# EasyVision-Ton/VMG

Hardware: AMD Instinct MI355X
Metric: LR-frames/s (train: forward+loss+backward+AdamW), VMG-REDS-few_levels 4x SR (higher is better)
Workload: dtype bf16; 1 GPU; VMG-REDS-few_levels train step, per-GPU batch 4x7x3x64x64 -> 4x SR (BASELINE configs[1]); global_batch=4, frames_per_clip=7, parallelism=dp1, launch=eager, recompute_chains=False, fp8_chains=False

## Files before the change

include/vmg_hip.h:

```cpp
#ifndef VMG_HIP_H
#define VMG_HIP_H

#include <stdint.h>

#ifdef __cplusplus
extern "C" {
#endif

#define VMG_F32 0
#define VMG_BF16 1

#define VMG_ACT_NONE 0
#define VMG_ACT_RELU 1
#define VMG_ACT_LRELU 2
#define VMG_ACT_GELU 3

#define VMG_CONV_GENERAL 0
#define VMG_CONV_KSPLIT 2
#define VMG_CONV_WS 3
#define VMG_CONV_LINEAR_WRES 4
#define VMG_CONV_WSTAT 6

const char* vmg_last_error(void);
int vmg_version(void);
// ... 131 lines not shown
int vmg_layernorm_bwd(int dtype, int ndy, const void* const* dy, const void* x, const float* mean, const float* rstd, const float* w,
                      const void* add, void* dx, float* dw, float* db, int64_t M, int C, void* ws, void* stream);

int vmg_space_depth_ln_fwd(int dtype, int mode, const void* x, const float* w, const float* b, void* y, float* mean, float* rstd, int N, int H,
                           int W, int cseg, float eps, void* stream);
int vmg_space_depth_ln_bwd(int dtype, int mode, const void* dy, const void* x, const float* mean, const float* rstd, const float* w, void* dx,
                           float* dw, float* db, int N, int H, int W, int cseg, void* ws, void* stream);

int64_t vmg_group_reduce_ws_bytes(void);
int vmg_group_reduce(int dtype, const void* a, const void* b, const void* c3, float* out, int G, int64_t R, int C, int mode, float scale,
                     float* ws, int64_t ws_bytes, void* stream);
int vmg_group_reduce3(int dtype, const void* a, const void* b0, const void* b1, const void* b2, float* out, int G, int64_t R, int C, float scale,
                      float* ws, int64_t ws_bytes, void* stream);
int vmg_tab_elementwise(int dtype, int op, const void* p0, const void* p1, const void* p2, const float* coef, const float* add, float s,
                        void* o0, void* o1, void* o2, int64_t rows, int64_t R, int C, void* stream);

#define VMG_GATE_TANH 0
#define VMG_GATE_SIGMOID_SYMM 1
#define VMG_GATE_RELU 2
#define VMG_GATE_GELU 3
#define VMG_GATE_SILU 4
int vmg_gate_fwd(int dtype, int form, int act, const void* a, const void* y, void* out, int64_t rows, int C, void* stream);
int vmg_gate_bwd(int dtype, int form, int act, const void* dout, const void* a, const void* y, void* da, void* dy, int64_t rows, int C, void* stream);
int vmg_gate_res_fwd(int dtype, int form, int act, const void* a, const void* y, const void* res, const float* coef, void* out, int64_t rows, int G,
                     int C, void* stream);
int vmg_gate_res_bwd(int dtype, int form, int act, const void* dout, const void* a, const void* y, const float* coef, void* da, void* dy,
                     int64_t rows, int G, int C, void* stream);

#define VMG_SHIFT_VECTOR 1
#define VMG_SHIFT_ELEMENT 2
int vmg_patch_shift_plan(int dtype, int Cs, int aligned16);
int vmg_patch_shift_fwd(int dtype, int sign, int act, const void* x, void* y, int N, int H, int W, int Cs, void* stream);
int vmg_patch_shift_bwd(int dtype, int sign, int act, const void* dy, const void* x, void* dx, int N, int H, int W, int Cs, void* stream);
int vmg_se_mlp2_fwd(const float* m, const float* w1, const float* b1, const float* w2, const float* b2, float* pre, float* out, int G, int C, int Hd,
                    void* stream);
int vmg_se_mlp2_bwd(const float* dout, const float* out, const float* m, const float* pre, const float* w1, const float* w2, float* dm, float* dw1,
                    float* db1, float* dw2, float* db2, float* ws, int G, int C, int Hd, float dm_scale, int accumulate, void* stream);
int vmg_group_reduce2(int dtype, const void* a, const void* b0, const void* b1, float* out, int G, int64_t R, int C, float scale, float* ws,
                      int64_t ws_bytes, void* stream);
int vmg_mix2_fwd(int dtype, const void* h, const void* w, const float* coef, void* y, int64_t rows, int64_t R, int C, void* stream);
int vmg_mix2_bwd(int dtype, const void* dy, const float* coef, const float* add, void* dh, void* dw, int64_t rows, int64_t R, int C, void* stream);

#define VMG_DWCONV_VECTOR 1
#define VMG_DWCONV_ELEMENT 2
#define VMG_DWCONV_PLAN_INTS 8
int vmg_dwconv3_plan(int dtype, int N, int H, int W, int C, int aligned16, int* plan);
int vmg_dwconv3_fwd(int dtype, int src_act, int out_act, const void* e, const float* w, const float* b, void* a, int N, int H, int W, int C, void* stream);
int vmg_dwconv3_bwd_data(int dtype, int src_act, int out_act, const void* da, const void* a, const void* e, const float* w, void* de, int N, int H, int W,
                         int C, void* stream);
int64_t vmg_dwconv3_wgrad_ws_bytes(int dtype, int N, int H, int W, int C);
int vmg_dwconv3_bwd_weight(int dtype, int src_act, int out_act, const void* da, const void* a, const void* e, float* dW, float* db, int N, int H, int W,
                           int C, int accumulate, void* ws, int64_t ws_bytes, void* stream);

int vmg_warp_bilinear_fwd(int dtype, const void* x, const float* flow, void* out, int N, int H, int W, int C, void* stream);
int vmg_warp_bilinear_bwd(int dtype, const void* x, const float* flow, const void* dy, void* dx_acc, float* dflow, int N, int H,
                          int W, int C, void* stream);
int vmg_warp_nearest_planes(const float* loc, const float* flow, float* out, int N, int K2, int H, int W, void* stream);
int vmg_flow_smooth(const float* in, float* out, int64_t planes, int H, int W, int r, int backward, void* stream);

int vmg_ltam_fwd(int dtype, const void* q, const void* const* keys, const void* const* vals, const float* loc, const float* rpe,
                 const float* decay, void* out, float* lse, int n, int h, int w, int c, int heads, int wh, int ww, int t, float scale,
                 void* stream);
int vmg_ltam_bwd(int dtype, const void* q, const void* const* keys, const void* const* vals, const float* loc, const float* rpe,
                 const float* decay, const void* out, const float* lse, const void* dout, void* dq, void* const* dk_acc,
                 void* const* dv_acc, float* drpe, int n, int h, int w, int c, int heads, int wh, int ww, int t, float scale,
                 void* stream);
int64_t vmg_ltam_tab_bytes(int t);
int vmg_ltam_fwd_tab(int dtype, const void* q, const void* const* keys, const void* const* vals, const float* loc, const float* rpe,
                     const float* decay, void* out, float* lse, int n, int h, int w, int c, int heads, int wh, int ww, int t, float scale,
                     void* ws, int64_t ws_bytes, void* stream);
int vmg_ltam_bwd_tab(int dtype, const void* q, const void* const* keys, const void* const* vals, const float* loc, const float* rpe,
                     const float* decay, const void* out, const float* lse, const void* dout, void* dq, void* const* dk_acc,
                     void* const* dv_acc, float* drpe, int n, int h, int w, int c, int heads, int wh, int ww, int t, float scale,
                     void* ws, int64_t ws_bytes, void* stream);

int vmg_ltam_max_fwd(int dtype, const void* q, const void* const* keys, const void* const* vals, const float* loc, void* out, int* idx,
                     float* score, int n, int h, int w, int c, int heads, int t, void* stream);
int vmg_ltam_max_bwd(int dtype, const void* q, const void* const* keys, const void* const* vals, const float* loc, const int* idx,
                     const void* dout, void* dq, void* const* dk_acc, void* const* dv_acc, int n, int h, int w, int c, int heads, int t,
                     void* stream);
int vmg_ltam_max_fwd_tab(int dtype, const void* q, const void* const* keys, const void* const* vals, const float* loc, void* out, int* idx,
                         float* score, int n, int h, int w, int c, int heads, int t, void* ws, int64_t ws_bytes, void* stream);
int vmg_ltam_max_bwd_tab(int dtype, const void* q, const void* const* keys, const void* const* vals, const float* loc, const int* idx,
                         const void* dout, void* dq, void* const* dk_acc, void* const* dv_acc, int n, int h, int w, int c, int heads, int t,
                         void* ws, int64_t ws_bytes, void* stream);

int vmg_prof_begin(vmg_ctx* ctx, int klass, int stride, int max_samples);
int vmg_prof_end(vmg_ctx* ctx, int64_t* launches_seen, int* samples, double* total_ms);
int vmg_prof_select_pixels(vmg_ctx* ctx, int64_t pixels);
double vmg_prof_null_interval_us(int reps, void* stream);

int vmg_morphfc_fwd(int axis, int chunk, const void* x, const void* relu_mask, const void* packed, const float* bias, void* out, void* tok_out,
                    int BT, int H, int W, int C, int Cp, int cout_tiles, int relu, float in_scale, float out_scale, void* stream);
int64_t vmg_morphfc_token_rows(int axis, int chunk, int BT, int H, int W);
enum { VMG_MORPHFC_PLAN_INTS = 8 };
int vmg_morphfc_plan(int axis, int chunk, int BT, int H, int W, int C, int Cp, int has_mask, int ncu, int* plan);
int64_t vmg_morph_token_rows(int axis, int chunk, int BT, int H, int W);
int vmg_morph_tokens_gather(int dtype, int axis, int chunk, const void* x, void* tok, int BT, int H, int W, int C, int Cp, int ld, void* stream);
int vmg_morph_tokens_scatter(int dtype, int axis, int chunk, const void* tok, void* out, int BT, int H, int W, int C, int Cp, int ld, void* stream);
int vmg_morph_tokens_route(int dtype, int chunk, int C, int ld, int aligned);

int vmg_win3d_attn_fwd(int dtype, const void* q, const void* kv, const float* bq, const float* bkv, const float* table, void* out, float* lse,
                       int B, int D, int H, int W, int C, int heads, int wt, int sd, int sh, int sw, void* stream);
int64_t vmg_win3d_attn_bwd_ws_bytes(int B, int D, int H, int W, int heads, int wt);
int vmg_win3d_attn_bwd(int dtype, const void* q, const void* kv, const float* bq, const float* bkv, const float* table, const void* out,
                       const float* lse, const void* d_out, void* dq, void* dkv, float* dtable, float* dbq, float* dbkv, void* ws, int B, int D, int H, int W,
// ... 122 lines not shown
```

vmg_amd/csrc/warp.hip:

```cpp
#include "common.h"

namespace {

__device__ __forceinline__ float unnorm_coord(float pix, float flow, int size) {
  const float g = __fadd_rn(pix, flow);
  const float denom = (float)(size - 1 > 1 ? size - 1 : 1);
  const float gn = __fsub_rn(__fdiv_rn(__fmul_rn(2.0f, g), denom), 1.0f);
  return __fmul_rn(__fdiv_rn(__fadd_rn(gn, 1.0f), 2.0f), (float)(size - 1));
}

__device__ __forceinline__ float clip_border(float v, int size, float* grad_mult) {
  const float hi = (float)(size - 1);
  if (v <= 0.f) { if (grad_mult) *grad_mult = 0.f; return 0.f; }
  if (v >= hi) { if (grad_mult) *grad_mult = 0.f; return hi; }
  if (grad_mult) *grad_mult = 1.f;
  return v;
}

template <typename T>
struct V16 {
  static constexpr int N = 16 / sizeof(T);
  T v[N];
};

// ... 58 lines not shown
    const float x1f = x0f + 1.f, y1f = y0f + 1.f;
    const float tx = ix - x0f, ty = iy - y0f;
    const float wnw = (x1f - ix) * (y1f - iy), wne = (ix - x0f) * (y1f - iy), wsw = (x1f - ix) * (iy - y0f), wse = (ix - x0f) * (iy - y0f);
    const bool vnw = y0 >= 0 && y0 < H && x0 >= 0 && x0 < W, vne = y0 >= 0 && y0 < H && x1 >= 0 && x1 < W;
    const bool vsw = y1 >= 0 && y1 < H && x0 >= 0 && x0 < W, vse = y1 >= 0 && y1 < H && x1 >= 0 && x1 < W;
    const long long ib = n * H * W * C;
    const long long onw = ib + ((long long)y0 * W + x0) * C, one = ib + ((long long)y0 * W + x1) * C;
    const long long osw = ib + ((long long)y1 * W + x0) * C, ose = ib + ((long long)y1 * W + x1) * C;
    float gix = 0.f, giy = 0.f;
    if constexpr (sizeof(T) == 2) {
      for (int cb = 0; cb < C; cb += 128) {
        const int cp = cb + 2 * lane;
        const bool in = cp < C;
        const long long own = pix * C;
        const int cl = in ? cp : 0;
        const wp_bf16x2 gp = *reinterpret_cast<const wp_bf16x2*>(dy + own + cl);
        const wp_bf16x2 xnw = *reinterpret_cast<const wp_bf16x2*>(x + (vnw ? onw : own) + cl), xne = *reinterpret_cast<const wp_bf16x2*>(x + (vne ? one : own) + cl);
        const wp_bf16x2 xsw = *reinterpret_cast<const wp_bf16x2*>(x + (vsw ? osw : own) + cl), xse = *reinterpret_cast<const wp_bf16x2*>(x + (vse ? ose : own) + cl);
        const float g0 = in ? (float)gp[0] : 0.f, g1 = in ? (float)gp[1] : 0.f;
        const int sl = lane >> 1;
        const float a0 = __shfl(g0, sl, 64), a1 = __shfl(g1, sl, 64), b0 = __shfl(g0, 32 + sl, 64), b1 = __shfl(g1, 32 + sl, 64);
        const float glo = (lane & 1) ? a1 : a0, ghi = (lane & 1) ? b1 : b0;
        const int clo = cb + lane, chi = cb + 64 + lane;
        auto corner = [&](long long o, float wgt, float sx, float sy, wp_bf16x2 xp) __attribute__((always_inline)) {
          if (clo < C) atomicAdd(dx_acc + o + clo, glo * wgt);
          if (chi < C) atomicAdd(dx_acc + o + chi, ghi * wgt);
          const float xv = (float)xp[0] * g0 + (float)xp[1] * g1;
          gix += xv * sx;
          giy += xv * sy;
        };
        if (vnw) corner(onw, wnw, -(1.f - ty), -(1.f - tx), xnw);
        if (vne) corner(one, wne, (1.f - ty), -tx, xne);
        if (vsw) corner(osw, wsw, -ty, (1.f - tx), xsw);
        if (vse) corner(ose, wse, ty, tx, xse);
      }
    } else {
      for (int c = lane; c < C; c += 64) {
        const float g = to_f32(dy[pix * C + c]);
        if (vnw) { atomicAdd(dx_acc + onw + c, g * wnw); const float xv = to_f32(x[onw + c]) * g; gix -= xv * (1.f - ty); giy -= xv * (1.f - tx); }
        if (vne) { atomicAdd(dx_acc + one + c, g * wne); const float xv = to_f32(x[one + c]) * g; gix += xv * (1.f - ty); giy -= xv * tx; }
        if (vsw) { atomicAdd(dx_acc + osw + c, g * wsw); const float xv = to_f32(x[osw + c]) * g; gix -= xv * ty; giy += xv * (1.f - tx); }
        if (vse) { atomicAdd(dx_acc + ose + c, g * wse); const float xv = to_f32(x[ose + c]) * g; gix += xv * ty; giy += xv * tx; }
      }
    }
    gix = wave_sum(gix);
    giy = wave_sum(giy);
    if (lane == 0) {
      dflow[pix * 2] = gix * gmx;
      dflow[pix * 2 + 1] = giy * gmy;
    }
  }
}

__global__ __launch_bounds__(256) void warp_nearest_planes_kernel(const float* __restrict__ loc, const float* __restrict__ flow,
                                                                  float* __restrict__ out, int N, int K2, int H, int W) {
  const long long total = (long long)N * H * W;
  for (long long pix = blockIdx.x * 256LL + threadIdx.x; pix < total; pix += (long long)gridDim.x * 256) {
    const int px = (int)(pix % W);
    const int py = (int)((pix / W) % H);
    const long long n = pix / ((long long)W * H);
    const float ix = clip_border(unnorm_coord((float)px, flow[pix * 2], W), W, nullptr);
    const float iy = clip_border(unnorm_coord((float)py, flow[pix * 2 + 1], H), H, nullptr);
    const int xn = (int)nearbyintf(ix), yn = (int)nearbyintf(iy);
    const bool ok = xn >= 0 && xn < W && yn >= 0 && yn < H;
    for (int k = 0; k < K2; ++k) {
      const long long plane = (n * K2 + k) * H * W;
      out[plane + (long long)py * W + px] = ok ? loc[plane + (long long)yn * W + xn] : 0.f;
    }
  }
}

int grid_for(long long total) {
  long long b = (total + 255) / 256;
  return (int)(b > 8192 ? 8192 : (b < 1 ? 1 : b));
}

__device__ __forceinline__ int fs_reflect(int p, int n) { return p < n ? p : 2 * (n - 1) - p; }

__global__ void flow_smooth_fwd_kernel(const float* __restrict__ in, float* __restrict__ out, long long planes, int H, int W, int r) {
  const long long total = planes * H * W;
  const float inv = 1.0f / (float)(r * r);
  for (long long i = blockIdx.x * (long long)blockDim.x + threadIdx.x; i < total; i += (long long)gridDim.x * blockDim.x) {
    const int x = (int)(i % W), y = (int)((i / W) % H);
    const float* pl = in + (i / ((long long)W * H)) * H * W;
    const int y0 = (y / r) * r, x0 = (x / r) * r;
    float s = 0.f;
    for (int dy = 0; dy < r; ++dy) {
      const float* row = pl + (long long)fs_reflect(y0 + dy, H) * W;
      for (int dx = 0; dx < r; ++dx) s += row[fs_reflect(x0 + dx, W)];
    }
    out[i] = s * inv;
  }
}

__global__ void flow_smooth_bwd_kernel(const float* __restrict__ dout, float* __restrict__ din, long long planes, int H, int W, int r) {
  const long long total = planes * H * W;
  const int hf = (H + r - 1) / r * r, wf = (W + r - 1) / r * r;
  const float inv = 1.0f / (float)(r * r);
  for (long long i = blockIdx.x * (long long)blockDim.x + threadIdx.x; i < total; i += (long long)gridDim.x * blockDim.x) {
    const int x = (int)(i % W), y = (int)((i / W) % H);
    const float* pl = dout + (i / ((long long)W * H)) * H * W;
    int py[2] = {y, 2 * (H - 1) - y}, px[2] = {x, 2 * (W - 1) - x};
    const int ny = (py[1] >= H && py[1] < hf) ? 2 : 1, nx = (px[1] >= W && px[1] < wf) ? 2 : 1;
    float acc = 0.f;
    for (int a = 0; a < ny; ++a) {
      const int y0 = (py[a] / r) * r;
      for (int b = 0; b < nx; ++b) {
        const int x0 = (px[b] / r) * r;
        float g = 0.f;
        for (int dy = 0; dy < r && y0 + dy < H; ++dy)
          for (int dx = 0; dx < r && x0 + dx < W; ++dx) g += pl[(long long)(y0 + dy) * W + x0 + dx];
        acc += g;
      }
    }
    din[i] = acc * inv;
  }
}

}

extern "C" int vmg_warp_bilinear_fwd(int dtype, const void* x, const float* flow, void* out, int N, int H, int W, int C, void* stream) {
  VMG_CHECK(dtype == VMG_F32 || dtype == VMG_BF16, "warp_fwd: bad dtype");
  VMG_CHECK(x && flow && out && N > 0 && H > 0 && W > 0 && C > 0, "warp_fwd: bad arguments");
  const int vn = dtype == VMG_BF16 ? 8 : 4;
  VMG_CHECK(C % vn == 0, "warp_fwd: C must be a multiple of %d", vn);
  VMG_CHECK(((uintptr_t)x | (uintptr_t)out) % 16 == 0, "warp_fwd: pointers must be 16-byte aligned");
  const long long total = (long long)N * H * W * (C / vn);
  hipStream_t st = (hipStream_t)stream;
  if (dtype == VMG_BF16) hipLaunchKernelGGL(warp_bilinear_fwd_kernel<bf16>, dim3(grid_for(total)), dim3(256), 0, st, (const bf16*)x, flow, (bf16*)out, N, H, W, C);
  else hipLaunchKernelGGL(warp_bilinear_fwd_kernel<float>, dim3(grid_for(total)), dim3(256), 0, st, (const float*)x, flow, (float*)out, N, H, W, C);
  VMG_LAUNCH_CHECK();
  return 0;
}

extern "C" int vmg_warp_bilinear_bwd(int dtype, const void* x, const float* flow, const void* dy, void* dx_acc, float* dflow, int N,
                                     int H, int W, int C, void* stream) {
  VMG_CHECK(dtype == VMG_F32 || dtype == VMG_BF16, "warp_bwd: bad dtype");
  VMG_CHECK(x && flow && dy && dx_acc && dflow && N > 0 && H > 0 && W > 0 && C > 0, "warp_bwd: bad arguments");
  const int vn = dtype == VMG_BF16 ? 8 : 4;
  VMG_CHECK(C % vn == 0, "warp_bwd: C must be a multiple of %d", vn);
  VMG_CHECK(((uintptr_t)x | (uintptr_t)dy | (uintptr_t)dx_acc) % 16 == 0, "warp_bwd: pointers must be 16-byte aligned");
  const long long total = (long long)N * H * W * 64;
  hipStream_t st = (hipStream_t)stream;
  if (dtype == VMG_BF16) {
    hipLaunchKernelGGL(warp_bilinear_bwd_kernel<bf16>, dim3(grid_for(total)), dim3(256), 0, st, (const bf16*)x, flow, (const bf16*)dy, (float*)dx_acc, dflow, N, H, W, C);
  } else {
    hipLaunchKernelGGL(warp_bilinear_bwd_kernel<float>, dim3(grid_for(total)), dim3(256), 0, st, (const float*)x, flow, (const float*)dy, (float*)dx_acc, dflow, N, H, W, C);
  }
  VMG_LAUNCH_CHECK();
  return 0;
}

extern "C" int vmg_warp_nearest_planes(const float* loc, const float* flow, float* out, int N, int K2, int H, int W, void* stream) {
  VMG_CHECK(loc && flow && out && N > 0 && K2 > 0 && H > 0 && W > 0, "warp_nearest: bad arguments");
  hipLaunchKernelGGL(warp_nearest_planes_kernel, dim3(grid_for((long long)N * H * W)), dim3(256), 0, (hipStream_t)stream, loc, flow, out, N, K2, H, W);
  VMG_LAUNCH_CHECK();
  return 0;
}

extern "C" int vmg_flow_smooth(const float* in, float* out, int64_t planes, int H, int W, int r, int backward, void* stream) {
  VMG_CHECK(in && out && planes > 0 && H > 0 && W > 0 && r >= 1, "flow_smooth: bad arguments");
  const int hf = (H + r - 1) / r * r, wf = (W + r - 1) / r * r;
  VMG_CHECK(hf - H < H && wf - W < W, "flow_smooth: the reflected padding must be smaller than the plane (as F.pad(mode='reflect') demands)");
  const long long total = planes * H * W;
  if (backward) hipLaunchKernelGGL(flow_smooth_bwd_kernel, dim3(grid_for(total)), dim3(256), 0, (hipStream_t)stream, in, out, (long long)planes, H, W, r);
  else hipLaunchKernelGGL(flow_smooth_fwd_kernel, dim3(grid_for(total)), dim3(256), 0, (hipStream_t)stream, in, out, (long long)planes, H, W, r);
  VMG_LAUNCH_CHECK();
  return 0;
}
```

vmg_amd/hip.py:

```python
from __future__ import annotations

import ctypes
import os
from ctypes import POINTER, c_char_p, c_float, c_int, c_int64, c_void_p

import torch

HERE = os.path.dirname(os.path.abspath(__file__))
LIB_PATH = os.environ.get("VMG_HIP_LIB") or os.path.join(HERE, "libvmg_hip.so")

F32, BF16 = 0, 1
ACT_NONE, ACT_RELU, ACT_LRELU, ACT_GELU = 0, 1, 2, 3
GATE_ACTS = {"tanh": 0, "sigmoid": 1, "relu": 2, "gelu": 3, "swish": 4}
SHIFT_VECTOR, SHIFT_ELEMENT = 1, 2
DWCONV_VECTOR, DWCONV_ELEMENT, DWCONV_PLAN_INTS = 1, 2, 8
CONV_GENERAL, CONV_KSPLIT, CONV_WS, CONV_LINEAR_WRES, CONV_WSTAT = 0, 2, 3, 4, 6
CONV_FAM_IGEMM, CONV_FAM_KSPLIT, CONV_FAM_WS, CONV_FAM_LINEAR_WRES, CONV_FAM_WSTAT = 1, 2, 3, 4, 5
CONV_PLAN_INTS = 11
MORPHFC_PLAN_INTS = 8
MORPH_ROUTE_ELEMENT, MORPH_ROUTE_LDS = 0, 1
WGRAD_V1, WGRAD_3, WGRAD_3B, WGRAD_L2, WGRAD_7 = 1, 2, 3, 4, 5


def wgrad_kernel_id(kind: int, a: int = 0, b: int = 0, c: int = 0) -> int:
    return kind << 24 | a << 16 | b << 8 | c


class HipError(RuntimeError):
    pass


class ConvDesc(ctypes.Structure):
    _fields_ = [
        ("dtype", c_int), ("ks", c_int), ("cout_tiles", c_int),
        ("N", c_int), ("H", c_int), ("W", c_int), ("Cout", c_int),
        ("nsrc", c_int),
        ("src", c_void_p * 4), ("src_ps", c_int64 * 4), ("src_ch", c_int * 4),
        ("packed", c_void_p), ("bias", c_void_p),
        ("out", c_void_p), ("out_ps", c_int64), ("out_pre", c_void_p),
        ("res", c_void_p), ("res_ps", c_int64),
        ("aux", c_void_p), ("aux_ps", c_int64),
        ("act", c_int), ("slope", c_float), ("alpha", c_float),
        ("actgrad", c_int), ("pixel_shuffle", c_int), ("mt", c_int), ("deep", c_int),
    ]


class ChainDesc(ctypes.Structure):
    _fields_ = [
        ("dtype", c_int), ("N", c_int), ("H", c_int), ("W", c_int), ("C", c_int), ("nblk", c_int), ("nsrc", c_int),
        ("src", c_void_p * 4), ("src_ps", c_int64 * 4), ("src_ch", c_int * 4),
        ("packed0", c_void_p), ("bias0", c_void_p), ("slope0", c_float), ("cout_tiles0", c_int), ("deep0", c_int),
        ("packed1", POINTER(c_void_p)), ("bias1", POINTER(c_void_p)), ("packed2", POINTER(c_void_p)), ("bias2", POINTER(c_void_p)),
        ("r_scaling", c_float), ("cout_tiles", c_int), ("deep", c_int),
        ("y", POINTER(c_void_p)), ("t", POINTER(c_void_p)), ("g_y", POINTER(c_void_p)), ("g_t", POINTER(c_void_p)),
    ]


class SpyModuleDesc(ctypes.Structure):
    _fields_ = [
        ("N", c_int), ("H", c_int), ("W", c_int),
        ("x", c_void_p), ("packed", c_void_p * 5), ("bias", c_void_p * 5), ("y", c_void_p * 4), ("out", c_void_p), ("dpre", c_void_p * 4),
    ]


class ConvQ8Desc(ctypes.Structure):
    _fields_ = [
        ("N", c_int), ("H", c_int), ("W", c_int), ("Cin", c_int), ("Cout", c_int),
        ("src", c_void_p), ("packed", c_void_p), ("bias", c_void_p),
        ("out", c_void_p), ("out_ps", c_int64), ("outq", c_void_p),
        ("res", c_void_p), ("res_ps", c_int64),
        ("act", c_int), ("slope", c_float), ("alpha", c_float),
    ]

# ... 35 lines not shown
                                  c_void_p, c_void_p]),
    "vmg_morphfc_fwd": (c_int, [c_int, c_int, c_void_p, c_void_p, c_void_p, c_void_p, c_void_p, c_void_p, c_int, c_int, c_int, c_int, c_int, c_int, c_int, c_float, c_float,
                                c_void_p]),
    "vmg_morphfc_token_rows": (c_int64, [c_int, c_int, c_int, c_int, c_int]),
    "vmg_morphfc_plan": (c_int, [c_int, c_int, c_int, c_int, c_int, c_int, c_int, c_int, c_int, POINTER(c_int)]),
    "vmg_morph_tokens_route": (c_int, [c_int, c_int, c_int, c_int, c_int]),
    "vmg_morph_token_rows": (c_int64, [c_int, c_int, c_int, c_int, c_int]),
    "vmg_morph_tokens_gather": (c_int, [c_int, c_int, c_int, c_void_p, c_void_p, c_int, c_int, c_int, c_int, c_int, c_int, c_void_p]),
    "vmg_morph_tokens_scatter": (c_int, [c_int, c_int, c_int, c_void_p, c_void_p, c_int, c_int, c_int, c_int, c_int, c_int, c_void_p]),
    "vmg_win3d_attn_fwd": (c_int, [c_int, c_void_p, c_void_p, c_void_p, c_void_p, c_void_p, c_void_p, c_void_p, c_int, c_int, c_int, c_int, c_int, c_int, c_int,
                                   c_int, c_int, c_int, c_void_p]),
    "vmg_win3d_attn_bwd": (c_int, [c_int, c_void_p, c_void_p, c_void_p, c_void_p, c_void_p, c_void_p, c_void_p, c_void_p, c_void_p, c_void_p, c_void_p, c_void_p,
                                   c_void_p, c_void_p, c_int, c_int, c_int, c_int, c_int, c_int, c_int, c_int, c_int, c_int, c_void_p]),
    "vmg_win3d_attn_bwd_ws_bytes": (c_int64, [c_int, c_int, c_int, c_int, c_int, c_int]),
    "vmg_conv_wgrad3_multi": (c_int, [c_int, c_int, c_void_p, c_void_p, c_int, c_int, c_int, c_int64, c_int, c_int64, c_int, c_void_p, c_int, c_int, c_int,
                                      c_void_p, c_void_p, c_void_p, c_int64, c_void_p]),
    "vmg_conv_wgrad3_variant": (c_int, [c_int]),
    "vmg_conv_wgrad_last_kernel": (c_int, []),
    "vmg_conv_wgrad_plan": (c_int, [c_int, c_int, c_int, c_int, c_int, c_int, c_int, c_int, c_int64, c_int, c_int64, c_int, c_int, c_int, c_int, c_int, c_int64,
                                    POINTER(c_int)]),
    "vmg_win3d_variant": (c_int, [c_int]),
    "vmg_linear_wgrad2_multi": (c_int, [c_int, c_int, c_void_p, c_void_p, c_int64, c_int64, c_int, c_int64, c_int, c_void_p, c_int, c_int, c_int,
                                        c_void_p, c_void_p, c_void_p, c_int64, c_void_p]),
    "vmg_replay_build": (c_void_p, [c_void_p, c_void_p, c_void_p]),
    "vmg_replay_kernel_info": (c_int, [c_void_p, c_int, c_void_p, c_void_p, c_void_p, c_void_p]),
    "vmg_replay_run": (c_int, [c_void_p, c_int, c_int, c_void_p]),
    "vmg_replay_destroy": (None, [c_void_p]),
    "vmg_pack_entry_bytes": (c_int, []),
    "vmg_pack_entry": (c_int, [c_void_p, c_int, c_int, c_void_p, c_int, c_int, c_int, c_int, c_int, c_int, c_void_p, c_void_p, c_int, c_int, c_void_p,
                               c_int]),
    "vmg_pack_run": (c_int, [c_void_p, c_int, c_int, c_void_p]),
    "vmg_group_reduce3": (c_int, [c_int, c_void_p, c_void_p, c_void_p, c_void_p, c_void_p, c_int, c_int64, c_int, ctypes.c_float, c_void_p, c_int64, c_void_p]),
    "vmg_group_reduce_ws_bytes": (c_int64, []),
    "vmg_se_mlp_fwd": (c_int, [c_void_p] * 7 + [c_int] * 6 + [c_void_p]),
    "vmg_se_mlp_bwd": (c_int, [c_void_p] * 12 + [c_int] * 6 + [ctypes.c_float, c_int, c_void_p]),
    "vmg_maxpool_fwd": (c_int, [c_int, c_void_p, c_void_p, c_void_p, c_int, c_int, c_int, c_int, c_int, c_void_p]),
    "vmg_maxpool_bwd": (c_int, [c_int, c_void_p, c_void_p, c_void_p, c_int, c_int, c_int, c_int, c_int, c_void_p]),
    "vmg_avgpool2_nhwc": (c_int, [c_int, c_void_p, c_void_p, c_int, c_int, c_int, c_int, c_void_p]),
    "vmg_upsample2x_ac_fwd": (c_int, [c_void_p, c_void_p, c_int, c_int, c_int, c_int, c_float, c_void_p]),
    "vmg_upsample2x_ac_bwd": (c_int, [c_void_p, c_void_p, c_int, c_int, c_int, c_int, c_float, c_void_p]),
    "vmg_spy_operand_fwd": (c_int, [c_int, c_void_p, c_void_p, c_void_p, c_void_p, c_int64, c_void_p]),
    "vmg_spy_operand_bwd": (c_int, [c_int, c_void_p, c_void_p, c_void_p, c_int64, c_void_p]),
    "vmg_spy_flow_add": (c_int, [c_int, c_void_p, c_void_p, c_void_p, c_int64, c_void_p]),
    "vmg_spy_prep": (c_int, [c_int, c_void_p, c_void_p, c_void_p, c_void_p, c_int64, c_int, c_int, c_void_p]),
    "vmg_spy_module_fwd": (c_int, [POINTER(SpyModuleDesc), c_void_p]),
    "vmg_spy_module_bwd": (c_int, [POINTER(SpyModuleDesc), c_void_p]),
    "vmg_space_depth_ln_fwd": (c_int, [c_int, c_int, c_void_p, c_void_p, c_void_p, c_void_p, c_void_p, c_void_p, c_int, c_int, c_int, c_int, c_float, c_void_p]),
    "vmg_space_depth_ln_bwd": (c_int, [c_int, c_int, c_void_p, c_void_p, c_void_p, c_void_p, c_void_p, c_void_p, c_void_p, c_void_p, c_int, c_int, c_int, c_int,
                                       c_void_p, c_void_p]),
    "vmg_conv_wgrad_batched": (c_int, [c_int, c_int, c_int, POINTER(c_void_p), POINTER(c_void_p), c_int, c_int, c_int, c_int64, c_int,
                                       c_int64, c_int, c_void_p, c_int, c_int, c_int, c_void_p, c_float, c_void_p]),
    "vmg_warp_bilinear_fwd": (c_int, [c_int, c_void_p, c_void_p, c_void_p, c_int, c_int, c_int, c_int, c_void_p]),
    "vmg_warp_bilinear_bwd": (c_int, [c_int, c_void_p, c_void_p, c_void_p, c_void_p, c_void_p, c_int, c_int, c_int, c_int, c_void_p]),
    "vmg_warp_nearest_planes": (c_int, [c_void_p, c_void_p, c_void_p, c_int, c_int, c_int, c_int, c_void_p]),
    "vmg_flow_smooth": (c_int, [c_void_p, c_void_p, c_int64, c_int, c_int, c_int, c_int, c_void_p]),
    "vmg_ltam_fwd": (c_int, [c_int, c_void_p, POINTER(c_void_p), POINTER(c_void_p), c_void_p, c_void_p, c_void_p, c_void_p, c_void_p,
                             c_int, c_int, c_int, c_int, c_int, c_int, c_int, c_int, c_float, c_void_p]),
    "vmg_ltam_bwd": (c_int, [c_int, c_void_p, POINTER(c_void_p), POINTER(c_void_p), c_void_p, c_void_p, c_void_p, c_void_p, c_void_p,
                             c_void_p, c_void_p, POINTER(c_void_p), POINTER(c_void_p), c_void_p, c_int, c_int, c_int, c_int, c_int,
                             c_int, c_int, c_int, c_float, c_void_p]),
    "vmg_ltam_tab_bytes": (c_int64, [c_int]),
    "vmg_ltam_fwd_tab": (c_int, [c_int, c_void_p, POINTER(c_void_p), POINTER(c_void_p), c_void_p, c_void_p, c_void_p, c_void_p, c_void_p,
                                 c_int, c_int, c_int, c_int, c_int, c_int, c_int, c_int, c_float, c_void_p, c_int64, c_void_p]),
    "vmg_ltam_bwd_tab": (c_int, [c_int, c_void_p, POINTER(c_void_p), POINTER(c_void_p), c_void_p, c_void_p, c_void_p, c_void_p, c_void_p,
                                 c_void_p, c_void_p, POINTER(c_void_p), POINTER(c_void_p), c_void_p, c_int, c_int, c_int, c_int, c_int,
                                 c_int, c_int, c_int, c_float, c_void_p, c_int64, c_void_p]),
    "vmg_ltam_max_fwd": (c_int, [c_int, c_void_p, POINTER(c_void_p), POINTER(c_void_p), c_void_p, c_void_p, c_void_p, c_void_p,
                                 c_int, c_int, c_int, c_int, c_int, c_int, c_void_p]),
    "vmg_ltam_max_bwd": (c_int, [c_int, c_void_p, POINTER(c_void_p), POINTER(c_void_p), c_void_p, c_void_p, c_void_p, c_void_p,
                                 POINTER(c_void_p), POINTER(c_void_p), c_int, c_int, c_int, c_int, c_int, c_int, c_void_p]),
    "vmg_ltam_max_fwd_tab": (c_int, [c_int, c_void_p, POINTER(c_void_p), POINTER(c_void_p), c_void_p, c_void_p, c_void_p, c_void_p,
                                     c_int, c_int, c_int, c_int, c_int, c_int, c_void_p, c_int64, c_void_p]),
    "vmg_ltam_max_bwd_tab": (c_int, [c_int, c_void_p, POINTER(c_void_p), POINTER(c_void_p), c_void_p, c_void_p, c_void_p, c_void_p,
                                     POINTER(c_void_p), POINTER(c_void_p), c_int, c_int, c_int, c_int, c_int, c_int, c_void_p, c_int64,
                                     c_void_p]),
    "vmg_charbonnier_edge_blocks": (c_int, [c_int64, c_int, c_int]),
    "vmg_charbonnier_edge_fwd": (c_int, [c_void_p, c_void_p, c_void_p, c_void_p, c_void_p, c_int64, c_int, c_int, c_float, c_void_p]),
    "vmg_charbonnier_edge_bwd": (c_int, [c_void_p, c_void_p, c_void_p, c_void_p, c_void_p, c_int64, c_int, c_int, c_float, c_float, c_float, c_void_p]),
    "vmg_adamw_flat": (c_int, [c_void_p, c_void_p, c_void_p, c_void_p, c_int64, c_void_p, c_float, c_float, c_float, c_void_p]),
    "vmg_q8_record_bytes": (c_int, [c_int]),
    "vmg_q8_quantize": (c_int, [c_void_p, c_int64, c_void_p, c_int64, c_int, c_void_p]),
    "vmg_convq8_pack_bytes": (c_int64, [c_int, c_int]),
    "vmg_convq8_pack": (c_int, [c_void_p, c_int, c_int, c_int, c_void_p, c_void_p]),
    "vmg_convq8_fwd": (c_int, [POINTER(ConvQ8Desc), c_void_p]),
    "vmg_resblock_chain_fwd_q8": (c_int, [POINTER(ChainQ8Desc), c_void_p]),
    "vmg_grad_clip_ws_bytes": (c_int64, []),
    "vmg_grad_clip_norm": (c_int, [c_void_p, c_int64, c_float, c_void_p, c_void_p, c_void_p]),
    "vmg_grad_pack_bf16": (c_int, [c_void_p, c_void_p, c_int64, c_float, c_void_p]),
    "vmg_grad_unpack_bf16": (c_int, [c_void_p, c_void_p, c_int64, c_void_p]),
    "vmg_tile_accumulate": (c_int, [c_int, c_void_p, c_void_p, c_void_p, c_int64, c_int, c_int, c_int, c_int, c_int, c_int, c_int, c_int, c_int,
                                    c_int, c_void_p]),
    "vmg_tile_finalize": (c_int, [c_void_p, c_void_p, c_void_p, c_void_p, c_int64, c_void_p]),
    "vmg_frame_metrics_ws_bytes": (c_int64, [c_int, c_int, c_int]),
    "vmg_frame_metrics": (c_int, [c_void_p, POINTER(c_int64), c_void_p, POINTER(c_int64), c_int, c_int, c_int, POINTER(ctypes.c_double), c_void_p, c_int64,
                                  c_void_p, c_void_p, c_void_p]),
    "vmg_bicubic_down": (c_int, [c_void_p, POINTER(c_int64), c_int, c_int, c_int, c_int, c_int, c_void_p, c_void_p]),
    "vmg_crop_batch": (c_int, [c_void_p, POINTER(c_int64), c_void_p, c_int, c_int, c_int, c_int, c_int, c_int, c_int, c_void_p, c_void_p]),
    "vmg_decay_weights": (c_int, [POINTER(c_void_p), POINTER(c_void_p), POINTER(c_int64), c_int, c_int, c_void_p]),
    "vmg_conv_debug_stamps": (c_int, [c_void_p]),
    "vmg_create": (c_void_p, [c_int]),
    "vmg_destroy": (c_int, [c_void_p]),
    "vmg_ctx_device": (c_int, [c_void_p]),
    "vmg_prof_select_pixels": (c_int, [c_void_p, c_int64]),
    "vmg_prof_null_interval_us": (ctypes.c_double, [c_int, c_void_p]),
    "vmg_conv_wgrad_ws_bytes": (c_int64, []),
    "vmg_conv_wgrad_batched_ws": (c_int, [c_int, c_int, c_int, POINTER(c_void_p), POINTER(c_void_p), c_int, c_int, c_int, c_int64, c_int,
# ... 98 lines not shown
```

vmg_amd/kernels.py:

```python
from __future__ import annotations

import collections
import ctypes
import os
import struct
from typing import Optional, Sequence, Tuple

import torch

from . import hip
from .hip import ConvDesc, HipError


def _intarr(v: Sequence[int]):
    return (ctypes.c_int * len(v))(*[int(x) for x in v])


def cout_tiles_for(cout: int, dtype: torch.dtype = torch.bfloat16, ks: int = 3) -> int:
    t = (cout + 15) // 16
    if t <= 1:
        return 1
    if ks == 7:
        return 2 if t == 2 else 4
    if t <= 4:
# ... 857 lines not shown


WGRAD_MULTI_PAIRS = 16


def _wgrad_multi(name: str, probs, dims: Sequence[int]):
    conv3 = len(dims) == 3
    M = dims[0] * dims[1] * dims[2] if conv3 else dims[0]
    xs0, dys0, dW0 = probs[0][:3]
    npairs = len(xs0)
    for xs, dys, dW, db, _ in probs:
        if len(xs) != npairs or len(dys) != npairs or dW.shape != dW0.shape or xs[0].dtype != torch.bfloat16:
            raise HipError(f"{name}: problems must share the shape; operands bf16")
        Cin, Cout, xps, dps, I_total = _wgrad_operands(name, xs, dys, dW, db, 3 if conv3 else 1, M, like=(xs0[0], dys0[0]), whole=True)
    entry = getattr(hip.lib(), "vmg_" + name)
    ws = _workspace("vmg_conv_wgrad_ws_bytes", dW0.device)
    for s in range(0, len(probs), 8):
        grp = probs[s:s + 8]
        n = len(grp)
        wa = (ctypes.c_void_p * n)(*[g[2].data_ptr() for g in grp])
        ba = (ctypes.c_void_p * n)(*[(g[3].data_ptr() if g[3] is not None else None) for g in grp])
        sa = (ctypes.c_float * n)(*[float(g[4]) for g in grp])
        for p0 in range(0, npairs, WGRAD_MULTI_PAIRS):
            p1 = min(npairs, p0 + WGRAD_MULTI_PAIRS)
            xa = (ctypes.c_void_p * (n * (p1 - p0)))(*[t.data_ptr() for g in grp for t in g[0][p0:p1]])
            da = (ctypes.c_void_p * (n * (p1 - p0)))(*[t.data_ptr() for g in grp for t in g[1][p0:p1]])
            hip.check(entry(n, p1 - p0, xa, da, *dims, xps, Cin, dps, Cout, wa, I_total, 0, 0, ba, sa, ws.data_ptr(), ws.numel(), hip.stream_ptr()),
                      "vmg_" + name)


def linear_wgrad2_multi(probs, M: int):
    _wgrad_multi("linear_wgrad2_multi", probs, (M,))


def conv_wgrad3_multi(probs, N: int, H: int, W: int):
    _wgrad_multi("conv_wgrad3_multi", probs, (N, H, W))


def _ptrs(ts):
    return (ctypes.c_void_p * len(ts))(*[t.data_ptr() for t in ts])


def warp_bilinear_forward(x: torch.Tensor, flow: torch.Tensor) -> torch.Tensor:
    hip.require_cuda(x, flow)
    n, h, w, c = x.shape
    if not x.is_contiguous() or flow.dtype != torch.float32 or not flow.is_contiguous() or tuple(flow.shape) != (n, h, w, 2):
        raise HipError("warp: x must be contiguous (n,h,w,c), flow contiguous fp32 (n,h,w,2)")
    out = torch.empty_like(x)
    hip.check(hip.lib().vmg_warp_bilinear_fwd(hip.dtype_code(x.dtype), x.data_ptr(), flow.data_ptr(), out.data_ptr(), n, h, w, c,
                                              hip.stream_ptr()), "vmg_warp_bilinear_fwd")
    return out


def warp_bilinear_backward(x: torch.Tensor, flow: torch.Tensor, dy: torch.Tensor):
    hip.require_cuda(x, flow, dy)
    n, h, w, c = x.shape
    if not x.is_contiguous() or flow.dtype != torch.float32 or not flow.is_contiguous() or tuple(flow.shape) != (n, h, w, 2):
        raise HipError("warp: x must be contiguous (n,h,w,c), flow contiguous fp32 (n,h,w,2)")
    if dy.dtype != x.dtype or tuple(dy.shape) != (n, h, w, c):
        raise HipError(f"warp_bilinear_backward: dy must have x's shape and dtype, got {tuple(dy.shape)} {dy.dtype}")
    dy = dy.contiguous()
    pooled = x.dtype != torch.float32 and (n * h * w * c) % 4 == 0
    dx_acc = ACC_POOL.take((n, h, w, c), x.device) if pooled else torch.zeros((n, h, w, c), dtype=torch.float32, device=x.device)
    dflow = torch.empty((n, h, w, 2), dtype=torch.float32, device=x.device)
    hip.check(hip.lib().vmg_warp_bilinear_bwd(hip.dtype_code(x.dtype), x.data_ptr(), flow.data_ptr(), dy.data_ptr(), dx_acc.data_ptr(),
                                              dflow.data_ptr(), n, h, w, c, hip.stream_ptr()), "vmg_warp_bilinear_bwd")
    if pooled:
        dx = cast_clear(dx_acc, x.dtype)
        ACC_POOL.give(dx_acc)
        return dx, dflow
    return dx_acc.to(x.dtype), dflow


def flow_smooth(x: torch.Tensor, r: int, backward: bool = False) -> torch.Tensor:
    hip.require_cuda(x)
    if x.dtype != torch.float32 or not x.is_contiguous() or x.dim() < 2:
        raise HipError("flow_smooth: contiguous fp32 (..., H, W) expected")
    H, W = x.shape[-2:]
    out = torch.empty_like(x)
    hip.check(hip.lib().vmg_flow_smooth(x.data_ptr(), out.data_ptr(), x.numel() // (H * W), H, W, int(r), 1 if backward else 0, hip.stream_ptr()), "vmg_flow_smooth")
    return out


def warp_nearest_planes(loc: torch.Tensor, flow: torch.Tensor) -> torch.Tensor:
    hip.require_cuda(loc, flow)
    n, k2, h, w = loc.shape
    if loc.dtype != torch.float32 or flow.dtype != torch.float32 or not flow.is_contiguous() or tuple(flow.shape) != (n, h, w, 2):
        raise HipError("warp_nearest_planes: fp32 loc (n,k2,h,w) and flow (n,h,w,2) expected")
    loc = loc.contiguous()
    out = torch.empty_like(loc)
    hip.check(hip.lib().vmg_warp_nearest_planes(loc.data_ptr(), flow.data_ptr(), out.data_ptr(), n, k2, h, w, hip.stream_ptr()),
              "vmg_warp_nearest_planes")
    return out


def _ltam_check_tables(rpe, decay, heads, wh, ww):
    wq = wh * ww
    if rpe.dtype != torch.float32 or decay.dtype != torch.float32 or not rpe.is_contiguous():
        raise HipError("ltam: rpe / decay must be fp32")
    if tuple(rpe.shape) != (heads, wq, wq):
        raise HipError(f"ltam: rpe must be (heads, wh*ww, wh*ww) = {(heads, wq, wq)}, got {tuple(rpe.shape)}")
    if decay.numel() != heads or not decay.is_contiguous():
        raise HipError(f"ltam: decay must hold {heads} contiguous values, got {tuple(decay.shape)}")


class LtamTables:
# ... 865 lines not shown
```

Before: 597.0 LR-frames/s.

## Add run-based bf16 warp backward kernel that merges adjacent-pixel scatter atomics

Adds a bilinear warp backward kernel for bf16 where each wavefront processes a run of 8 horizontally adjacent pixels. It carries the right-column (NE/SE) contributions forward and merges them with the next pixel's left-column (NW/SW) contributions when they hit the same source location, which cuts the number of atomicAdds into dx_acc. It also loads bf16 pairs per lane and unrolls two pixels to overlap loads. The kernel is selected automatically when C is a multiple of 8 and at most 256. The cost is more register pressure and less parallelism, since there is one wave per run instead of one per pixel.

Result: no change. 600.9 LR-frames/s, median of 6 (+0.7%).

```diff
diff --git a/include/vmg_hip.h b/include/vmg_hip.h
--- a/include/vmg_hip.h
+++ b/include/vmg_hip.h
@@ -207,6 +207,9 @@
 int vmg_dwconv3_bwd_weight(int dtype, int src_act, int out_act, const void* da, const void* a, const void* e, float* dW, float* db, int N, int H, int W,
                            int C, int accumulate, void* ws, int64_t ws_bytes, void* stream);
 
+#define VMG_WARP_BWD_PIXEL 0
+#define VMG_WARP_BWD_RUN 1
+int vmg_warp_bwd_route(int dtype, int N, int H, int W, int C);
 int vmg_warp_bilinear_fwd(int dtype, const void* x, const float* flow, void* out, int N, int H, int W, int C, void* stream);
 int vmg_warp_bilinear_bwd(int dtype, const void* x, const float* flow, const void* dy, void* dx_acc, float* dflow, int N, int H,
                           int W, int C, void* stream);
diff --git a/vmg_amd/csrc/warp.hip b/vmg_amd/csrc/warp.hip
--- a/vmg_amd/csrc/warp.hip
+++ b/vmg_amd/csrc/warp.hip
@@ -134,6 +134,131 @@
   }
 }
 
+constexpr int WR_RUN = 8, WR_U = 2, WR_MAXCB = 2;
+
+struct WrPix {
+  long long pix;
+  float ix, iy, gmx, gmy;
+  int y0, x0;
+  bool live;
+};
+
+template <int R, int U, int MAXCB>
+__global__ __launch_bounds__(256) void warp_bilinear_bwd_run_kernel(const bf16* __restrict__ x, const float* __restrict__ flow,
+                                                                   const bf16* __restrict__ dy, float* __restrict__ dx_acc,
+                                                                   float* __restrict__ dflow, int N, int H, int W, int C) {
+  static_assert(R % U == 0, "the unroll must divide the run");
+  const int lane = threadIdx.x & 63;
+  const int runs_x = (W + R - 1) / R;
+  const long long nruns = (long long)N * H * runs_x;
+  auto emit = [&](long long o, int cb, float lo, float hi) __attribute__((always_inline)) {
+    if (cb + lane < C) atomicAdd(dx_acc + o + cb + lane, lo);
+    if (cb + 64 + lane < C) atomicAdd(dx_acc + o + cb + 64 + lane, hi);
+  };
+  for (long long run = blockIdx.x * 4LL + __builtin_amdgcn_readfirstlane(threadIdx.x >> 6); run < nruns; run += (long long)gridDim.x * 4) {
+    const int px0 = (int)(run % runs_x) * R;
+    const long long row = run / runs_x;
+    const int py = (int)(row % H);
+    const long long ib = (row / H) * H * W * C;
+    bool pt = false, pb = false;
+    long long pto = 0, pbo = 0;
+    float ptv[MAXCB][2], pbv[MAXCB][2];
+    for (int k0 = 0; k0 < R && px0 + k0 < W; k0 += U) {
+      WrPix p[U];
+      float gix[U], giy[U];
+#pragma unroll
+      for (int u = 0; u < U; ++u) {
+        const int px = px0 + k0 + u, pxc = min(px, W - 1);
+        p[u].pix = row * W + pxc;
+        const float fx = flow[p[u].pix * 2], fy = flow[p[u].pix * 2 + 1];
+        p[u].ix = clip_border(unnorm_coord((float)pxc, fx, W), W, &p[u].gmx);
+        p[u].iy = clip_border(unnorm_coord((float)py, fy, H), H, &p[u].gmy);
+        p[u].x0 = (int)floorf(p[u].ix), p[u].y0 = (int)floorf(p[u].iy);
+        p[u].live = px < W;
+        gix[u] = giy[u] = 0.f;
+      }
+      bool qt = pt, qb = pb;
+      long long qto = pto, qbo = pbo;
+#pragma unroll
+      for (int b = 0; b < MAXCB; ++b) {
+        const int cb = b * 128;
+        if (cb >= C) break;
+        const int cp = cb + 2 * lane;
+        const bool in = cp < C;
+        const int cl = in ? cp : 0;
+        wp_bf16x2 gp[U], xnw[U], xne[U], xsw[U], xse[U];
+#pragma unroll
+        for (int u = 0; u < U; ++u) {
+          const int y0 = p[u].y0, x0 = p[u].x0, y1 = y0 + 1, x1 = x0 + 1;
+          const bool vy0 = y0 >= 0 && y0 < H, vy1 = y1 >= 0 && y1 < H, vx0 = x0 >= 0 && x0 < W, vx1 = x1 >= 0 && x1 < W;
+          const long long own = p[u].pix * C + cl, onw = ib + ((long long)y0 * W + x0) * C + cl, osw = onw + (long long)W * C;
+          gp[u] = *reinterpret_cast<const wp_bf16x2*>(dy + own);
+          xnw[u] = *reinterpret_cast<const wp_bf16x2*>(x + (vy0 && vx0 ? onw : own));
+          xne[u] = *reinterpret_cast<const wp_bf16x2*>(x + (vy0 && vx1 ? onw + C : own));
+          xsw[u] = *reinterpret_cast<const wp_bf16x2*>(x + (vy1 && vx0 ? osw : own));
+          xse[u] = *reinterpret_cast<const wp_bf16x2*>(x + (vy1 && vx1 ? osw + C : own));
+        }
+        qt = pt, qb = pb, qto = pto, qbo = pbo;
+#pragma unroll
+        for (int u = 0; u < U; ++u) {
+          if (!p[u].live) continue;
+          const float g0 = in ? (float)gp[u][0] : 0.f, g1 = in ? (float)gp[u][1] : 0.f;
+          const int sl = lane >> 1;
+          const float a0 = __shfl(g0, sl, 64), a1 = __shfl(g1, sl, 64), b0 = __shfl(g0, 32 + sl, 64), b1 = __shfl(g1, 32 + sl, 64);
+          const float glo = (lane & 1) ? a1 : a0, ghi = (lane & 1) ? b1 : b0;
+          const float ix = p[u].ix, iy = p[u].iy;
+          const int y0 = p[u].y0, x0 = p[u].x0, y1 = y0 + 1, x1 = x0 + 1;
+          const float x0f = (float)x0, y0f = (float)y0, x1f = x0f + 1.f, y1f = y0f + 1.f;
+          const float tx = ix - x0f, ty = iy - y0f;
+          const float wnw = (x1f - ix) * (y1f - iy), wne = (ix - x0f) * (y1f - iy), wsw = (x1f - ix) * (iy - y0f), wse = (ix - x0f) * (iy - y0f);
+          const bool vy0 = y0 >= 0 && y0 < H, vy1 = y1 >= 0 && y1 < H, vx0 = x0 >= 0 && x0 < W, vx1 = x1 >= 0 && x1 < W;
+          const long long onw = ib + ((long long)y0 * W + x0) * C, osw = onw + (long long)W * C;
+          auto left = [&](bool valid, long long o, float wgt, bool pend, long long po, float (&pv)[2]) __attribute__((always_inline)) {
+            const float lo = __fmul_rn(glo, wgt), hi = __fmul_rn(ghi, wgt);
+            if (pend && valid && po == o) {
+              emit(o, cb, __fadd_rn(pv[0], lo), __fadd_rn(pv[1], hi));
+            } else {
+              if (pend) emit(po, cb, pv[0], pv[1]);
+              if (valid) emit(o, cb, lo, hi);
+            }
+          };
+          left(vy0 && vx0, onw, wnw, qt, qto, ptv[b]);
+          left(vy1 && vx0, osw, wsw, qb, qbo, pbv[b]);
+          qt = vy0 && vx1, qb = vy1 && vx1, qto = onw + C, qbo = osw + C;
+          ptv[b][0] = __fmul_rn(glo, wne), ptv[b][1] = __fmul_rn(ghi, wne);
+          pbv[b][0] = __fmul_rn(glo, wse), pbv[b][1] = __fmul_rn(ghi, wse);
+          auto grad = [&](bool valid, float sx, float sy, wp_bf16x2 xp) __attribute__((always_inline)) {
+            if (!valid) return;
+            const float xv = (float)xp[0] * g0 + (float)xp[1] * g1;
+            gix[u] += xv * sx;
+            giy[u] += xv * sy;
+          };
+          grad(vy0 && vx0, -(1.f - ty), -(1.f - tx), xnw[u]);
+          grad(vy0 && vx1, (1.f - ty), -tx, xne[u]);
+          grad(vy1 && vx0, -ty, (1.f - tx), xsw[u]);
+          grad(vy1 && vx1, ty, tx, xse[u]);
+        }
+      }
+      pt = qt, pb = qb, pto = qto, pbo = qbo;
+#pragma unroll
+      for (int u = 0; u < U; ++u) {
+        if (!p[u].live) continue;
+        const float sx = wave_sum(gix[u]), sy = wave_sum(giy[u]);
+        if (lane == 0) {
+          dflow[p[u].pix * 2] = sx * p[u].gmx;
+          dflow[p[u].pix * 2 + 1] = sy * p[u].gmy;
+        }
+      }
+    }
+#pragma unroll
+    for (int b = 0; b < MAXCB; ++b) {
+      if (b * 128 >= C) break;
+      if (pt) emit(pto, b * 128, ptv[b][0], ptv[b][1]);
+      if (pb) emit(pbo, b * 128, pbv[b][0], pbv[b][1]);
+    }
+  }
+}
+
 __global__ __launch_bounds__(256) void warp_nearest_planes_kernel(const float* __restrict__ loc, const float* __restrict__ flow,
                                                                   float* __restrict__ out, int N, int K2, int H, int W) {
   const long long total = (long long)N * H * W;
@@ -215,6 +340,11 @@
   return 0;
 }
 
+extern "C" int vmg_warp_bwd_route(int dtype, int N, int H, int W, int C) {
+  if ((dtype != VMG_F32 && dtype != VMG_BF16) || N < 1 || H < 1 || W < 1 || C < 1) return -1;
+  return (dtype == VMG_BF16 && C % 8 == 0 && C <= 128 * WR_MAXCB) ? VMG_WARP_BWD_RUN : VMG_WARP_BWD_PIXEL;
+}
+
 extern "C" int vmg_warp_bilinear_bwd(int dtype, const void* x, const float* flow, const void* dy, void* dx_acc, float* dflow, int N,
                                      int H, int W, int C, void* stream) {
   VMG_CHECK(dtype == VMG_F32 || dtype == VMG_BF16, "warp_bwd: bad dtype");
@@ -224,7 +354,11 @@
   VMG_CHECK(((uintptr_t)x | (uintptr_t)dy | (uintptr_t)dx_acc) % 16 == 0, "warp_bwd: pointers must be 16-byte aligned");
   const long long total = (long long)N * H * W * 64;
   hipStream_t st = (hipStream_t)stream;
-  if (dtype == VMG_BF16) {
+  if (vmg_warp_bwd_route(dtype, N, H, W, C) == VMG_WARP_BWD_RUN) {
+    const long long runs = (long long)N * H * cdiv(W, WR_RUN);
+    hipLaunchKernelGGL((warp_bilinear_bwd_run_kernel<WR_RUN, WR_U, WR_MAXCB>), dim3(grid_for(runs * 64)), dim3(256), 0, st, (const bf16*)x, flow, (const bf16*)dy,
+                       (float*)dx_acc, dflow, N, H, W, C);
+  } else if (dtype == VMG_BF16) {
     hipLaunchKernelGGL(warp_bilinear_bwd_kernel<bf16>, dim3(grid_for(total)), dim3(256), 0, st, (const bf16*)x, flow, (const bf16*)dy, (float*)dx_acc, dflow, N, H, W, C);
   } else {
     hipLaunchKernelGGL(warp_bilinear_bwd_kernel<float>, dim3(grid_for(total)), dim3(256), 0, st, (const float*)x, flow, (const float*)dy, (float*)dx_acc, dflow, N, H, W, C);
diff --git a/vmg_amd/hip.py b/vmg_amd/hip.py
--- a/vmg_amd/hip.py
+++ b/vmg_amd/hip.py
@@ -19,6 +19,7 @@
 CONV_PLAN_INTS = 11
 MORPHFC_PLAN_INTS = 8
 MORPH_ROUTE_ELEMENT, MORPH_ROUTE_LDS = 0, 1
+WARP_BWD_PIXEL, WARP_BWD_RUN = 0, 1
 WGRAD_V1, WGRAD_3, WGRAD_3B, WGRAD_L2, WGRAD_7 = 1, 2, 3, 4, 5
 
 
@@ -160,6 +161,7 @@
                                        c_int64, c_int, c_void_p, c_int, c_int, c_int, c_void_p, c_float, c_void_p]),
     "vmg_warp_bilinear_fwd": (c_int, [c_int, c_void_p, c_void_p, c_void_p, c_int, c_int, c_int, c_int, c_void_p]),
     "vmg_warp_bilinear_bwd": (c_int, [c_int, c_void_p, c_void_p, c_void_p, c_void_p, c_void_p, c_int, c_int, c_int, c_int, c_void_p]),
+    "vmg_warp_bwd_route": (c_int, [c_int, c_int, c_int, c_int, c_int]),
     "vmg_warp_nearest_planes": (c_int, [c_void_p, c_void_p, c_void_p, c_int, c_int, c_int, c_int, c_void_p]),
     "vmg_flow_smooth": (c_int, [c_void_p, c_void_p, c_int64, c_int, c_int, c_int, c_int, c_void_p]),
     "vmg_ltam_fwd": (c_int, [c_int, c_void_p, POINTER(c_void_p), POINTER(c_void_p), c_void_p, c_void_p, c_void_p, c_void_p, c_void_p,
diff --git a/vmg_amd/kernels.py b/vmg_amd/kernels.py
--- a/vmg_amd/kernels.py
+++ b/vmg_amd/kernels.py
@@ -933,6 +933,16 @@
     return out
 
 
+WARP_BWD_ROUTES = {hip.WARP_BWD_PIXEL: "pixel", hip.WARP_BWD_RUN: "run"}
+
+
+def warp_bwd_route(dtype: torch.dtype, n: int, h: int, w: int, c: int) -> str:
+    r = hip.lib().vmg_warp_bwd_route(hip.dtype_code(dtype), int(n), int(h), int(w), int(c))
+    if r not in WARP_BWD_ROUTES:
+        raise HipError(f"warp_bwd_route: no route for {dtype}, ({n}, {h}, {w}, {c})")
+    return WARP_BWD_ROUTES[r]
+
+
 def warp_bilinear_backward(x: torch.Tensor, flow: torch.Tensor, dy: torch.Tensor):
     hip.require_cuda(x, flow, dy)
     n, h, w, c = x.shape
```
